# vaibhawvipul/taper

Measured on AMD Instinct MI355X. Metric: MNIST samples/sec fwd+bwd+step, higher is better.
Workload: dtype f32; 1 GPU; mlp_784-128-10_b64; per_gpu_batch=64, global_batch=64, parallelism=single, comm=none, graph_record_steps=11577

## Files before the change

### include/taper_hip.h

```cpp
#ifndef TAPER_HIP_H
#define TAPER_HIP_H

#include <stddef.h>
#include <stdint.h>

#ifdef __cplusplus
extern "C" {
#endif

typedef struct th_ctx th_ctx;
typedef struct th_graph th_graph;
typedef struct th_event th_event;
typedef struct th_comm th_comm;

typedef struct th_adam_fuse {
    float *d_p, *d_m, *d_v;
    const int32_t *d_t;
    const float *d_lr;
    float beta1, beta2, eps, weight_decay;
} th_adam_fuse;

typedef struct th_adam_slice {
    const float *d_g;
    int64_t n;
// ... 44 lines not shown
                  int accumulate_mask);
int th_linear_bwd_adam(th_ctx *ctx, const float *d_x, const float *d_w, const float *d_dy, const float *d_relu_y,
                       float *d_dx, float *d_dw, float *d_db, int batch, int in_features, int out_features,
                       int accumulate_mask, const th_adam_fuse *w_fuse, const th_adam_fuse *b_fuse);
int th_linear_bwd_adam_ex(th_ctx *ctx, const float *d_x, const float *d_w, const float *d_dy, const float *d_relu_y,
                          float *d_dx, float *d_dw, float *d_db, int batch, int in_features, int out_features,
                          int accumulate_mask, const th_adam_fuse *w_fuse, const th_adam_fuse *b_fuse,
                          const th_adam_slice *extra, int n_extra);
int th_linear_bwd_dx_epilogue_rows(int batch, int in_features, int out_features);
int th_linear_bwd_separate_products(int batch, int in_features, int out_features, int with_dx, int with_dw, int dx_epilogue);
int th_linear_bwd_adam_ex2(th_ctx *ctx, const float *d_x, const float *d_w, const float *d_dy, const float *d_relu_y, float *d_dx,
                           float *d_dw, float *d_db, int batch, int in_features, int out_features, int accumulate_mask,
                           const th_adam_fuse *w_fuse, const th_adam_fuse *b_fuse, const th_adam_slice *extra, int n_extra, int mask_dx,
                           float *d_dx_colpart);

int th_linear_xent_head(th_ctx *ctx, const float *d_h, const float *d_w, const float *d_bias, const float *d_targets,
                        int batch, int in_features, int classes, float *d_logits, float *d_loss, float *d_ncorrect,
                        float *d_dh, float *d_dw, float *d_db, float *d_metrics, int64_t metrics_capacity,
                        int64_t *d_state, int64_t advance, int32_t *d_adam_tick, const th_adam_fuse *w_fuse,
                        const th_adam_fuse *b_fuse);
int th_linear_xent_head_masked(th_ctx *ctx, const float *d_h, const float *d_w, const float *d_bias, const float *d_targets,
                               int batch, int in_features, int classes, float *d_logits, float *d_loss, float *d_ncorrect,
                               float *d_dh, float *d_dw, float *d_db, float *d_metrics, int64_t metrics_capacity,
                               int64_t *d_state, int64_t advance, int32_t *d_adam_tick, const th_adam_fuse *w_fuse,
                               const th_adam_fuse *b_fuse, int mask_dh_by_h);

int th_linear_xent_wide(th_ctx *ctx, const float *d_x, const float *d_w, const float *d_bias, const float *d_targets,
                        int batch, int in_features, int classes, float *d_loss, float *d_ncorrect,
                        float *d_dx, float *d_dw, float *d_db, float *d_metrics, int64_t metrics_capacity,
                        int64_t *d_state, int64_t advance, int32_t *d_adam_tick);
int th_linear_xent_wide_ex(th_ctx *ctx, const float *d_x, const float *d_w, const float *d_bias, const float *d_targets, int batch,
                           int in_features, int classes, float *d_loss, float *d_ncorrect, float *d_dx, float *d_dw, float *d_db,
                           float *d_metrics, int64_t metrics_capacity, int64_t *d_state, int64_t advance, int32_t *d_adam_tick,
                           float *d_colsum_masked);
int th_bias_from_colsum_adam(th_ctx *ctx, const float *d_colsum, float *d_gb, int c, int hw, const th_adam_fuse *b_fuse,
                             const th_adam_slice *extra, int n_extra);
typedef struct th_wide_fuse {
    th_adam_fuse w, b, conv_b;
    float *d_conv_gb;
    int conv_c, conv_hw;
} th_wide_fuse;
int th_linear_xent_wide_fused(th_ctx *ctx, const float *d_x, const float *d_w, const float *d_bias, const float *d_targets, int batch,
                              int in_features, int classes, float *d_loss, float *d_ncorrect, float *d_dw, float *d_db,
                              float *d_metrics, int64_t metrics_capacity, int64_t *d_state, int64_t advance, int32_t *d_adam_tick,
                              float *d_colsum_masked, const th_wide_fuse *fuse);

int th_mlp_tail_supported(int batch, int in_features, int hidden, int classes, int need_dx);
int th_mlp_tail(th_ctx *ctx, const float *d_x, const float *d_h, const float *d_w2, const float *d_b2,
                const float *d_targets, int batch, int in_features, int hidden, int classes,
                float *d_loss, float *d_ncorrect, float *d_dw1, float *d_db1, float *d_dw2, float *d_db2,
                const float *d_w1, float *d_dx,
                float *d_metrics, int64_t metrics_capacity, int64_t *d_state, int64_t advance,
                const th_adam_fuse *w1_fuse, const th_adam_fuse *b1_fuse);

typedef struct th_mlp3_layer {
    const float *d_w, *d_b;
    float *d_dw, *d_db;
    const th_adam_fuse *w_fuse, *b_fuse;
    int out_features;
} th_mlp3_layer;
typedef struct th_mlp3_gap {
    const float *d_cnt;
    float *d_gb;
    int hw;
    const th_adam_fuse *b_fuse;
} th_mlp3_gap;
int th_mlp3_supported(int batch, int in_features, int h1, int h2, int classes);
int th_mlp3_xent(th_ctx *ctx, const float *d_x, const float *d_targets, int batch, int in_features, const th_mlp3_layer *layers,
                 float *d_dx, float *d_loss, float *d_ncorrect, float *d_metrics, int64_t metrics_capacity, int64_t *d_state,
                 int64_t advance, int32_t *d_tick, const th_mlp3_gap *gap);

typedef struct th_row_source {
    const float *d_rows;
    const float *d_labels;
    const int32_t *d_indices;
    const int64_t *d_cursor;
    int64_t n_indices;
    int64_t n_rows;
} th_row_source;
int th_mlp2_xent_supported(int batch, int in_features, int hidden, int classes, int64_t n_rows);
int th_mlp2_set_max_ksplit(th_ctx *ctx, int max_ksplit);
int th_mlp2_xent(th_ctx *ctx, const th_row_source *src, int batch, int in_features, int hidden, int classes, const float *d_w1,
                 const float *d_b1, const float *d_w2, const float *d_b2, float *d_dw1, float *d_db1, float *d_dw2, float *d_db2,
                 float *d_loss, float *d_ncorrect, float *d_metrics, int64_t metrics_capacity, int64_t *d_state, int64_t advance,
                 int32_t *d_tick, const th_adam_fuse *w1_fuse, const th_adam_fuse *b1_fuse, const th_adam_fuse *w2_fuse,
                 const th_adam_fuse *b2_fuse);

int th_mlp2_xent_deep_supported(int batch, int in_features, int h1, int h2, int classes, int64_t n_rows);
int th_mlp2_xent_deep(th_ctx *ctx, const th_row_source *src, int batch, int in_features, const th_mlp3_layer *layers, float *d_loss,
                      float *d_ncorrect, float *d_metrics, int64_t metrics_capacity, int64_t *d_state, int64_t advance, int32_t *d_tick);

int th_add(th_ctx *ctx, const float *d_a, const float *d_b, float *d_out, size_t n);
int th_sub(th_ctx *ctx, const float *d_a, const float *d_b, float *d_out, size_t n);
int th_mul(th_ctx *ctx, const float *d_a, const float *d_b, float *d_out, size_t n);
int th_div(th_ctx *ctx, const float *d_a, const float *d_b, float *d_out, size_t n);
int th_axpy(th_ctx *ctx, float alpha, const float *d_x, float *d_y, size_t n);
int th_mul_bwd(th_ctx *ctx, const float *d_gout, const float *d_other, float *d_g, size_t n);
int th_div_bwd(th_ctx *ctx, const float *d_gout, const float *d_a, const float *d_b, float *d_ga, float *d_gb, size_t n);
int th_add_scalar_dev(th_ctx *ctx, const float *d_scalar, float divisor, float *d_g, size_t n);

int th_relu_fwd(th_ctx *ctx, const float *d_x, float *d_y, size_t n);
int th_relu_bwd(th_ctx *ctx, const float *d_x, const float *d_gout, float *d_gin, size_t n, int accumulate);
int th_sigmoid_fwd(th_ctx *ctx, const float *d_x, float *d_y, size_t n);
int th_sigmoid_bwd(th_ctx *ctx, const float *d_y, const float *d_gout, float *d_gin, size_t n);
int th_exp_fwd(th_ctx *ctx, const float *d_x, float *d_y, size_t n);
int th_log_fwd(th_ctx *ctx, const float *d_x, float *d_y, size_t n);
// ... 234 lines not shown
```

### taper_amd/csrc/common.h

```cpp
#pragma once

#include <hip/hip_runtime.h>

#include <cstdarg>
#include <cstdint>
#include <cstdio>
#include <array>
#include <atomic>
#include <map>
#include <string>
#include <unordered_map>
#include <unordered_set>
#include <vector>

#include "../../include/taper_hip.h"
#include "../../include/taper_hip_debug.h"

namespace th {

void set_error(const char *fmt, ...);

#define TH_HIP(expr)                                                                         \
    do {                                                                                     \
        hipError_t e_ = (expr);                                                              \
// ... 35 lines not shown
constexpr int kNumCU = 256;
constexpr int kNumXCD = 8;

static inline int ceil_div(long a, long b) { return (int)((a + b - 1) / b); }

__device__ __forceinline__ void lds_barrier() {
    __builtin_amdgcn_fence(__ATOMIC_RELEASE, "workgroup", "local");
    __builtin_amdgcn_s_barrier();
    __builtin_amdgcn_fence(__ATOMIC_ACQUIRE, "workgroup", "local");
}

enum : int32_t { TH_DEVERR_NONE = 0, TH_DEVERR_TARGET_OOB = 1 };
static __device__ __attribute__((unused)) int32_t *g_err_word;
__device__ __forceinline__ void raise_target_oob(long cls, int classes) {
    int32_t *w = g_err_word;
    if (!w) return;
    w[1] = (int32_t)(cls > 0x7fffffffL ? 0x7fffffffL : cls);
    w[2] = classes;
    __threadfence_system();
    w[0] = TH_DEVERR_TARGET_OOB;
}
typedef int (*err_bind_fn)(int32_t *);
struct ErrBindReg { explicit ErrBindReg(err_bind_fn f); };
#define TH_USES_DEVICE_ERRORS()                                                                                        \
    namespace {                                                                                                        \
    int th_err_bind_here(int32_t *p) { return hipMemcpyToSymbol(HIP_SYMBOL(th::g_err_word), &p, sizeof(p)) == hipSuccess ? 0 : 1; } \
    th::ErrBindReg th_err_reg_here(th_err_bind_here);                                                                  \
    }

static inline int ew_grid(size_t n_items, int block) {
    long g = (long)((n_items + block - 1) / block);
    long cap = (long)kNumCU * 8;
    return (int)(g < 1 ? 1 : (g > cap ? cap : g));
}

}

struct th_ctx {
    int device = 0;
    hipStream_t stream = nullptr;
    std::multimap<size_t, void *> free_blocks;
    std::unordered_map<void *, size_t> block_size;
    std::unordered_set<void *> graph_owned;
    std::unordered_set<void *> graph_owned_freed;
    size_t bytes_reserved = 0, bytes_in_use = 0;
    bool capturing = false;
    std::vector<void *> capture_blocks;
    std::multimap<size_t, void *> capture_free;
    std::map<std::array<int, 8>, void *> conv_plans;
    int32_t *err_word = nullptr;
    int m2_max_ksplit = 8;
    const uint32_t *update_guard = nullptr;
    uint32_t *update_step_word = nullptr;
    unsigned *m2_arrive = nullptr;
};

struct th_graph {
    th_ctx *ctx = nullptr;
    hipGraph_t graph = nullptr;
    hipGraphExec_t exec = nullptr;
    std::vector<void *> blocks;
};

struct th_event {
    hipEvent_t ev = nullptr;
};
```

### taper_amd/csrc/host/taper.h

```cpp
#pragma once

#include <algorithm>
#include <cstdint>
#include <functional>
#include <map>
#include <memory>
#include <random>
#include <stdexcept>
#include <string>
#include <vector>

#include "../../../include/taper_hip.h"

namespace taper {

struct Error : std::runtime_error {
    explicit Error(const std::string &m) : std::runtime_error(m) {}
};
void th_check(int rc, const char *what);
#define TAPER_ASSERT(cond, msg)                       \
    do {                                              \
        if (!(cond)) throw ::taper::Error(msg);       \
    } while (0)

// ... 787 lines not shown
};

struct Metrics {
    std::vector<float> train_loss, train_acc, val_loss, val_acc, epoch_times;
    std::string last_line() const;
    std::string summary() const;
    void print_last() const;
    void plot_summary() const;
};

std::string format_f32_display(float v);

enum class StepForm { Mlp2Rows, ChainMlp3, Mlp3, ChainHead, MlpTail, LinearHead, LinearWide, Layered };
struct StepPlan {
    StepForm form = StepForm::Layered;
    size_t prefix = 0;
    Linear *linear[3] = {};
    std::vector<ConvStage> stages;
    bool fused_adam = false;
    bool pool_bias = false;
    bool conv_chain = false;
    bool exchange = false;
    void key(std::vector<uintptr_t> *out) const;
};

class Trainer {
   public:
    std::shared_ptr<Module> model;
    std::shared_ptr<Adam> optimizer;
    std::shared_ptr<Communicator> comm;
    Shape sample_shape;
    std::string device = "hip:gfx950";
    size_t graph_chunk = 128;
    int fuse_head = 2;
    bool fuse_adam = true;
    Trainer(std::shared_ptr<Module> m, std::shared_ptr<Adam> o) : model(std::move(m)), optimizer(std::move(o)) {}

    void train_step(const Tensor &images, const Tensor &labels, float *loss_out, float *acc_out);
    void check_comm() const;
    void check_batchnorm_comm() const;
    EpochResult train_epoch(DataLoader &loader);
    EpochResult evaluate(DataLoader &loader);
    EpochResult train_epoch_graph(DataLoader &loader, size_t max_steps = 0);
    std::shared_ptr<LRScheduler> scheduler;
    Metrics metrics;
    void fit(DataLoader &train_loader, DataLoader &val_loader, size_t epochs, bool verbose, bool graph = true);
    void save_checkpoint(const std::string &path) const;
    void load_checkpoint(const std::string &path);
    void save_optimizer_state(const std::string &path) const;
    void load_optimizer_state(const std::string &path);
    ~Trainer();

   private:
    void enqueue_steps(const float *d_images, const float *d_labels, const int32_t *d_indices, int64_t n_indices,
                       size_t batch, size_t steps);
    void enqueue_compute(const StepPlan &plan, float *d_xb, float *d_yb, size_t batch, const th_row_source *rows = nullptr);
    StepPlan plan_step(size_t batch, int64_t n_rows) const;
    void drop_graphs();
    std::vector<std::pair<size_t, th_graph *>> graphs_;
    std::vector<std::pair<size_t, th_graph *>> whole_graphs_;
    bool graph_capture_failed_ = false;
    std::vector<size_t> whole_capture_failed_;
    std::vector<uintptr_t> graph_key_;
    std::shared_ptr<Buffer> xb_, yb_, state_, metrics_, step_loss_, step_ncorrect_;
    QATWeightPass qat_pass_;
    bool has_qat() const;
    size_t metrics_cap_ = 0;
};

}
```

### taper_amd/csrc/host/trainer.cpp

```cpp
#include <algorithm>
#include <chrono>
#include <cmath>
#include <cstdio>
#include <cstdlib>
#include <cstring>
#include <fstream>

#include "nn_internal.h"
#include "../../../include/taper_hip_debug.h"

namespace taper {
MNISTDataset MNISTDataset::from_host(const std::vector<float> &images, const std::vector<float> &labels, bool train) {
    TAPER_ASSERT(images.size() == labels.size() * 784, "MNISTDataset: images must be [N,784]");
    MNISTDataset d;
    d.images = Tensor(images, {labels.size(), 784});
    d.labels = Tensor(labels, {labels.size()});
    d.train = train;
    return d;
}

MNISTDataset MNISTDataset::from_u8(const std::vector<uint8_t> &pixels, const std::vector<uint8_t> &labels, bool train) {
    TAPER_ASSERT(pixels.size() == labels.size() * 784, "MNISTDataset: pixels must be [N,784]");
    th_ctx *ctx = Device::ctx();
    MNISTDataset d;
// ... 334 lines not shown
            for (Linear *l : plan.linear)
                if (l) {
                    w.push_back(l->weight);
                    b.push_back(l->bias);
                }
            loss = mlp2_cross_entropy(*rows, batch, w, b, &ncorrect, &sink);
            break;
        }
        case StepForm::ChainMlp3:
        case StepForm::Mlp3: {
            const Tensor w3[3] = {L[0]->weight, L[1]->weight, L[2]->weight}, b3[3] = {L[0]->bias, L[1]->bias, L[2]->bias};
            loss = plan.form == StepForm::ChainMlp3 ? conv_chain_mlp3_cross_entropy(xin, plan.stages, w3, b3, y, &ncorrect, &sink)
                                                    : mlp3_cross_entropy(seq->forward_prefix(xin, plan.prefix), w3, b3, y, &ncorrect, &sink);
            break;
        }
        case StepForm::ChainHead:
            loss = conv_chain_head_cross_entropy(xin, plan.stages, L[0]->weight, L[0]->bias, y, &ncorrect, &sink);
            break;
        case StepForm::MlpTail: {
            Tensor xh = seq->forward_prefix(xin, plan.prefix);
            if (plan.fused_adam) adam->set_carry_deferred(true);
            loss = mlp_tail_cross_entropy(xh, L[0]->weight, L[0]->bias, L[1]->weight, L[1]->bias, y, &ncorrect, &sink);
            break;
        }
        case StepForm::LinearHead:
        case StepForm::LinearWide: {
            adam->flush_deferred();
            Tensor h = seq->forward_prefix(xin, plan.prefix);
            loss = plan.form == StepForm::LinearHead ? linear_cross_entropy(h, L[0]->weight, L[0]->bias, y, &ncorrect, &sink)
                                                     : linear_cross_entropy_wide(h, L[0]->weight, L[0]->bias, y, &ncorrect, &sink);
            break;
        }
        case StepForm::Layered: {
            adam->flush_deferred();
            qat_pass_.run(*model);
            Tensor h = seq ? seq->forward_prefix(xin, plan.prefix) : model->forward(xin);
            for (size_t i = plan.prefix; seq && i < seq->layers.size(); ++i) h = seq->layers[i]->forward(h);
            loss = cross_entropy_loss(h, y, &ncorrect, &sink);
            break;
        }
    }
    loss.backward();
    if (plan.exchange) {
        optimizer->step();
    } else if (!(comm && optimizer->step_reduced(*comm))) {
        reduce_grads(*this);
        optimizer->step();
        optimizer->set_step_guard(nullptr);
    }
    optimizer->zero_grad();
    adam->set_carry_deferred(false);
}

void Trainer::enqueue_steps(const float *d_images, const float *d_labels, const int32_t *d_indices, int64_t n_indices,
                            size_t batch, size_t steps) {
    int64_t *state = reinterpret_cast<int64_t *>(state_->d);
    struct Guard {
        Guard(const uint32_t *w, uint32_t *step) { TH(th_ctx_set_update_guard(Device::ctx(), w, step)); }
        ~Guard() { th_ctx_set_update_guard(Device::ctx(), nullptr, nullptr); }
    } guard(comm && comm->is_p2p() ? comm->error_word() : nullptr, comm && comm->is_p2p() ? comm->step_word() : nullptr);
    const StepPlan plan = plan_step(batch, d_indices ? n_indices : (int64_t)batch);
    if (plan.form == StepForm::Mlp2Rows) {
        const th_row_source rows{d_images, d_labels, d_indices, d_indices ? state + 1 : nullptr, d_indices ? n_indices : 0,
                                 d_indices ? n_indices : (int64_t)batch};
        for (size_t s = 0; s < steps; ++s) enqueue_compute(plan, nullptr, nullptr, batch, &rows);
    } else if (d_indices == nullptr) {
        enqueue_compute(plan, const_cast<float *>(d_images), const_cast<float *>(d_labels), batch);
    } else {
        TH(th_gather_batch(Device::ctx(), d_images, d_labels, d_indices, n_indices, state + 1, (int)(batch * steps), 784, xb_->d,
                           yb_->d));
        for (size_t s = 0; s < steps; ++s) enqueue_compute(plan, xb_->d + s * batch * 784, yb_->d + s * batch, batch);
    }
    optimizer->flush_deferred();
}

void Trainer::check_batchnorm_comm() const {
    if (!comm) return;
    std::vector<BatchNorm2d *> bns;
    batchnorm_modules(*model, &bns);
    TAPER_ASSERT(bns.empty(), "BatchNorm2d: data-parallel training of a model with batch normalisation is not supported (statistics are per rank)");
}

bool Trainer::has_qat() const {
    std::vector<const QATModule *> mods;
    qat_modules(*model, &mods, false);
    for (size_t i = 0; i < mods.size(); ++i)
        for (size_t j = i + 1; j < mods.size(); ++j)
            TAPER_ASSERT(mods[i] != mods[j], "QAT: the model holds the same QAT layer twice; the Trainer does not train a shared QAT layer");
    return !mods.empty();
}

void Trainer::drop_graphs() {
    for (auto &g : graphs_) th_graph_destroy(g.second);
    graphs_.clear();
    for (auto &g : whole_graphs_) th_graph_destroy(g.second);
    whole_graphs_.clear();
    whole_capture_failed_.clear();
}

EpochResult Trainer::train_epoch_graph(DataLoader &loader, size_t max_steps) {
    th_ctx *ctx = Device::ctx();
    static const bool trace = std::getenv("TAPER_TRACE_EPOCH") != nullptr;
    const auto t_enter = std::chrono::steady_clock::now();
    auto us_since = [&](std::chrono::steady_clock::time_point t0) { return std::chrono::duration<double, std::micro>(std::chrono::steady_clock::now() - t0).count(); };
    loader.reset();
    const MNISTDataset &ds = loader.dataset();
    const size_t n = ds.len(), bs = loader.batch_size();
    size_t nb = loader.num_batches();
    if (max_steps && max_steps < nb) nb = max_steps;
    const size_t n_full = std::min(nb, n / bs);
    const size_t rem_rows = nb > n_full ? n - n_full * bs : 0;
    const StepPlan plan = plan_step(bs, (int64_t)n), rem_plan = rem_rows ? plan_step(rem_rows, (int64_t)n) : StepPlan{};
    const bool full_in_place = plan.form == StepForm::Mlp2Rows;
    const size_t chunk = full_in_place ? std::max<size_t>(graph_chunk, 1) : std::max<size_t>(std::min<size_t>(graph_chunk, ((size_t)1 << 26) / (bs * 784)), 1);
    const float *d_img = ds.images.dptr(), *d_lab = ds.labels.dptr();
    const int32_t *d_idx = (!loader.shuffled() && bs >= n && nb == 1) ? nullptr : loader.d_indices();
    const size_t stage_rows = std::max(full_in_place ? (size_t)0 : chunk * bs, (rem_rows && rem_plan.form != StepForm::Mlp2Rows) ? rem_rows : (size_t)0);
    if (d_idx && stage_rows && (!xb_ || xb_->n < stage_rows * 784)) {
        drop_graphs();
        xb_ = Buffer::alloc(stage_rows * 784);
        yb_ = Buffer::alloc(stage_rows);
    }
    if (!state_) state_ = Buffer::alloc(4);
    if (metrics_cap_ < loader.num_batches() + 1) {
        drop_graphs();
        metrics_cap_ = loader.num_batches() + 1;
        metrics_ = Buffer::alloc_host(2 * metrics_cap_);
    }
    std::vector<uintptr_t> key{(uintptr_t)d_img, (uintptr_t)d_lab, (uintptr_t)d_idx, (uintptr_t)n, (uintptr_t)bs, (uintptr_t)comm.get(),
                               (uintptr_t)model.get(), (uintptr_t)optimizer.get(), (uintptr_t)optimizer->flat().p_arena->d,
                               (uintptr_t)optimizer->flat().g_arena->d, (uintptr_t)(xb_ ? xb_->d : nullptr), (uintptr_t)metrics_->d};
    plan.key(&key);
    for (size_t d : sample_shape) key.push_back((uintptr_t)d);
    for (float h : {optimizer->beta1(), optimizer->beta2(), optimizer->eps(), optimizer->weight_decay()}) {
        uint32_t bits;
        std::memcpy(&bits, &h, sizeof bits);
        key.push_back(bits);
    }
    key.push_back((uintptr_t)full_backward());
    {
        uintptr_t h = 1469598103934665603ull;
        for (const Tensor &p : optimizer->flat().params) h = (h ^ (uintptr_t)(p.get_requires_grad() ? 2 : 1)) * 1099511628211ull;
        key.push_back(h);
    }
    {
        std::vector<const QATModule *> mods, active;
        qat_modules(*model, &mods, false);
        qat_modules(*model, &active, true);
        if (!mods.empty()) {
            qat_pass_.sync(active);
            key.push_back((uintptr_t)qat::enabled() | (uintptr_t)qat::is_training() << 1);
            key.push_back((uintptr_t)qat_pass_.generation());
        }
        for (const QATModule *q : mods)
            key.push_back((uintptr_t)q->active() | (uintptr_t)q->config.activations << 1 | (uintptr_t)q->config.qtype << 2);
    }
    {
        std::vector<BatchNorm2d *> bns;
        batchnorm_modules(*model, &bns);
        for (const BatchNorm2d *b : bns) key.push_back((uintptr_t)0xb0 | (uintptr_t)b->is_training());
    }
    if (!graphs_.empty() && graph_key_ != key) drop_graphs();

    size_t done = 0;
    th_graph *whole = nullptr;
    if (nb == n_full && !graph_capture_failed_ && !(std::getenv("TAPER_NO_GRAPH") && std::getenv("TAPER_NO_GRAPH")[0] == '1'))
        for (auto &g : whole_graphs_)
            if (g.first == n_full) whole = g.second;
    const double us_prep = us_since(t_enter);
    if (!whole) TH(th_fill_f32(ctx, state_->d, 0.f, 4));
    const double us_fill = us_since(t_enter);
    if (whole) {
        TH(th_graph_launch(ctx, whole));
        done = n_full;
    }
    auto have = [&](size_t steps) {
        for (auto &g : graphs_)
            if (g.first == steps) return true;
        return false;
    };
    if (!graph_capture_failed_ && std::getenv("TAPER_NO_GRAPH") && std::getenv("TAPER_NO_GRAPH")[0] == '1') graph_capture_failed_ = true;
    if (comm && !graph_capture_failed_ && std::getenv("TAPER_DP_EAGER") && std::getenv("TAPER_DP_EAGER")[0] == '1')
        graph_capture_failed_ = true;
    std::vector<size_t> want;
    for (size_t steps = chunk;; steps /= 2) {
        if (steps < 1) steps = 1;
        if (!((steps > 1 && n_full < steps + 1) || have(steps)) && std::find(want.begin(), want.end(), steps) == want.end())
            want.push_back(steps);
        if (steps == 1) break;
    }
    if (!whole && !want.empty() && n_full > 0 && !graph_capture_failed_) {
        enqueue_steps(d_img, d_lab, d_idx, (int64_t)n, bs, 1);
        done = 1;
        for (size_t steps : want) {
            TH(th_graph_begin(ctx));
            th_graph *g = nullptr;
            try {
                enqueue_steps(d_img, d_lab, d_idx, (int64_t)n, bs, steps);
                TH(th_graph_end(ctx, &g));
            } catch (const std::exception &e) {
                if (!g) th_graph_end(ctx, &g);
                if (g) th_graph_destroy(g);
                if (!comm) throw;
                fprintf(stderr, "taper: step capture with the communicator failed (%s); running data-parallel steps eagerly\n", e.what());
                graph_capture_failed_ = true;
                break;
            }
            graphs_.emplace_back(steps, g);
        }
        std::sort(graphs_.begin(), graphs_.end(), [](const auto &x, const auto &y) { return x.first > y.first; });
        graph_key_ = key;
    }
    if (!whole) {
        const size_t tail = n_full - done > 0 ? (n_full - done) % chunk : 0;
        size_t exact = 0;
        for (auto &g : graphs_) exact += (g.first & (g.first - 1)) != 0 ? 1 : 0;
        if (tail > 2 && (tail & (tail - 1)) != 0 && !have(tail) && have(1) && exact < 4 && !graph_capture_failed_ &&
            graph_key_ == key) {
            TH(th_graph_begin(ctx));
            th_graph *g = nullptr;
            try {
                enqueue_steps(d_img, d_lab, d_idx, (int64_t)n, bs, tail);
                TH(th_graph_end(ctx, &g));
                graphs_.emplace_back(tail, g);
                std::sort(graphs_.begin(), graphs_.end(), [](const auto &x, const auto &y) { return x.first > y.first; });
            } catch (const std::exception &e) {
                fprintf(stderr, "taper: capturing a %zu-step remainder graph failed (%s); the ladder graphs serve it\n", tail, e.what());
                if (!g) th_graph_end(ctx, &g);
                if (g) th_graph_destroy(g);
                if (auto *adam = dynamic_cast<Adam *>(optimizer.get())) {
                    adam->set_carry_deferred(false);
                    adam->drop_step_bookkeeping();
                }
                optimizer->zero_grad();
                Tape::reset();
                if (!comm) throw;
            }
        }
    }
    if (!whole && done == 0 && nb == n_full && n_full >= 2 && have(n_full) && whole_graphs_.size() < 4 && !graph_capture_failed_ && graph_key_ == key &&
        std::find(whole_capture_failed_.begin(), whole_capture_failed_.end(), n_full) == whole_capture_failed_.end()) {
        TH(th_graph_begin(ctx));
        th_graph *g = nullptr;
        try {
            TH(th_fill_f32(ctx, state_->d, 0.f, 4));
            enqueue_steps(d_img, d_lab, d_idx, (int64_t)n, bs, n_full);
            TH(th_graph_end(ctx, &g));
            whole_graphs_.emplace_back(n_full, g);
            TH(th_graph_launch(ctx, g));
            done = n_full;
        } catch (const std::exception &e) {
            fprintf(stderr, "taper: capturing a whole-call graph of %zu steps failed (%s); reset + replay stay two launches\n", n_full, e.what());
            whole_capture_failed_.push_back(n_full);
            if (!g) th_graph_end(ctx, &g);
            if (g) th_graph_destroy(g);
            if (auto *adam = dynamic_cast<Adam *>(optimizer.get())) {
                adam->set_carry_deferred(false);
                adam->drop_step_bookkeeping();
            }
            optimizer->zero_grad();
            Tape::reset();
            if (!comm) throw;
        }
    }
    while (done < n_full) {
        bool launched = false;
        for (auto &g : graphs_) {
            if (done + g.first <= n_full) {
                TH(th_graph_launch(ctx, g.second));
                done += g.first;
                launched = true;
                break;
            }
        }
        if (!launched) {
            enqueue_steps(d_img, d_lab, d_idx, (int64_t)n, bs, 1);
            ++done;
        }
    }
    if (nb > n_full) {
        const size_t rem = n - n_full * bs;
        enqueue_steps(d_img, d_lab, d_idx, (int64_t)n, rem, 1);
    }
    loader.advance(std::min(n, nb * bs));

    const double us_enqueued = us_since(t_enter);
    Device::sync();
    check_comm();
    if (trace) fprintf(stderr, "taper trace: train_epoch_graph %zu steps (%s%s%s): state reset enqueued at %.1f - %.1f us, all enqueued after %.1f us, stream idle after %.1f us\n", nb,
                       step_form_names[(int)plan.form], rem_rows ? ", last batch " : "", rem_rows ? step_form_names[(int)rem_plan.form] : "", us_prep, us_fill, us_enqueued, us_since(t_enter));
    const float *mt = metrics_->d;
    EpochResult r;
    r.num_batches = nb;
    float total_loss = 0.f;
    for (size_t s = 0; s < nb; ++s) {
        const size_t b = (s < n_full) ? bs : n - n_full * bs;
        const float acc = mt[2 * s + 1] / (float)b;
        r.total_correct += (size_t)(acc * (float)b);
        r.total_samples += b;
// ... 13 lines not shown
```

### taper_amd/csrc/mlp_tail.hip

```cpp
#include "tail_dev.h"
#include "dp_dev.h"

TH_USES_DEVICE_ERRORS()

namespace th {

struct TailArgs {
    const float *x, *h, *w2, *b2, *targets;
    int batch, in_f, hid, c;
    float *loss, *ncorrect, *dw1, *db1, *dw2, *db2;
    float *metrics;
    int64_t capacity;
    int64_t *state;
    int64_t advance;
    AdamDev w1_adam, b1_adam;
    int n_dw, n_head, tiles_m, groups;
    const float *w1;
    float *dx;
    int xgroups;
    DpDev dp;
    int32_t *dp_tick;
};

#ifdef TH_PROFILE
__device__ long long g_tail_prof[2][16];
#define TAIL_STAMP(i)                                                                         \
    do {                                                                                      \
        __builtin_amdgcn_sched_barrier(0);                                                    \
        if (threadIdx.x == 0 && (blockIdx.x == 0 || blockIdx.x == a.n_head))                  \
            g_tail_prof[blockIdx.x == 0 ? 0 : 1][i] = wall_clock64();                         \
        __builtin_amdgcn_sched_barrier(0);                                                    \
    } while (0)
__global__ void tail_prof_mark_kernel(int i) { g_tail_prof[0][i] = g_tail_prof[1][i] = wall_clock64(); }
#else
#define TAIL_STAMP(i) do { } while (0)
#endif

template <int KS, int TN>
__global__ __launch_bounds__(256) void mlp_tail_kernel(TailArgs a) {
    __shared__ float red[4][TN][64][4];
    __shared__ float tr[4][16][17];
    __shared__ float sc[4][36];
    const int t = threadIdx.x, lane = t & 63, wave = t >> 6, r16 = lane & 15, g4 = lane >> 4;
    const int bid = blockIdx.x;
    TAIL_STAMP(0);
    const bool head_role = bid < a.n_head;
    int tile_m, grp = 0;
    if (!head_role) {
        const int b2 = bid - a.n_head;
        const int tt = (b2 & 7) * (a.n_dw >> 3) + (b2 >> 3);
        if (tt >= a.tiles_m * a.groups) return;
        tile_m = tt % a.tiles_m;
        grp = tt / a.tiles_m;
    } else {
        tile_m = bid;
        if (tile_m >= a.tiles_m) return;
    }
    const int hid = a.hid, C = a.c, in_f = a.in_f, B = a.batch;
    const int hcol = tile_m * 16 + r16;
    const bool hcol_ok = hcol < hid;
    const int col0 = grp * 16 * TN;
    const bool lead = head_role && tile_m == 0;

    const bool any_w = a.w1_adam.p != nullptr, any_b = a.db1 && a.b1_adam.p != nullptr;
    const int32_t w_t = any_w ? sload(a.w1_adam.t) : 1, b_t = any_b ? sload(a.b1_adam.t) : 1;
    const float w_lr = any_w ? sload(a.w1_adam.lr) : 0.f, b_lr = any_b ? sload(a.b1_adam.lr) : 0.f;
    const int Cm1 = C - 1, hid4 = hid - 4, hcol_c = min(hcol, hid - 1);
// ... 277 lines not shown
    float lg[4], dl[4], nll_row;
    int bi;
#pragma unroll
    for (int i = 0; i < 4; ++i) lg[i] = (g4 * 4 + i < C) ? ((ax[i] + ay[i]) + (az[i] + aw[i])) + b2v[i] : -INFINITY;
    tail_row_softmax(lg, g4, C, tf, 1.0f / (float)B, dl, nll_row, bi);

    floatx4 accx[TX];
#pragma unroll
    for (int tx = 0; tx < TX; ++tx) accx[tx] = floatx4{0.f, 0.f, 0.f, 0.f};
#pragma unroll
    for (int th0 = 0; th0 < KS; th0 += TH_BLK) {
        float w2t[TH_BLK][4], w1v[TH_BLK][TX][4];
#pragma unroll
        for (int t = 0; t < TH_BLK; ++t)
#pragma unroll
            for (int s = 0; s < 4; ++s) {
                w2t[t][s] = ldg_b(a.w2, cls_off[s] + (th0 + t) * 64);
#pragma unroll
                for (int tx = 0; tx < TX; ++tx)
                    w1v[t][tx][s] = tx_ok[tx] ? ldg_b(a.w1, w1_off + ((th0 + t) * 16 + s) * in_f * 4u + tx * 64) : 0.f;
            }
#pragma unroll
        for (int t = 0; t < TH_BLK; ++t) {
            floatx4 dht = {0.f, 0.f, 0.f, 0.f};
#pragma unroll
            for (int s = 0; s < 4; ++s) dht = __builtin_amdgcn_mfma_f32_16x16x4f32(w2t[t][s], dl[s], dht, 0, 0, 0);
            const float4 hq = hv[th0 + t];
            const float m[4] = {hq.x > 0.f ? dht[0] : 0.f, hq.y > 0.f ? dht[1] : 0.f, hq.z > 0.f ? dht[2] : 0.f, hq.w > 0.f ? dht[3] : 0.f};
#pragma unroll
            for (int s = 0; s < 4; ++s)
#pragma unroll
                for (int tx = 0; tx < TX; ++tx) accx[tx] = __builtin_amdgcn_mfma_f32_16x16x4f32(m[s], w1v[t][tx][s], accx[tx], 0, 0, 0);
        }
    }
    const unsigned x_off = ((unsigned)(r0 + g4 * 4) * in_f + col0 + r16) * 4u;
#pragma unroll
    for (int tx = 0; tx < TX; ++tx) {
        if (!tx_ok[tx]) continue;
#pragma unroll
        for (int i = 0; i < 4; ++i) *reinterpret_cast<float *>(reinterpret_cast<char *>(a.dx) + x_off + i * in_f * 4u + tx * 64) = accx[tx][i];
    }
}

template <int KS, int TN, bool HAS_DX, int NW, int DPNR = 0>
__global__ __launch_bounds__(64 * NW) void mlp_tail_exact_kernel(TailArgs a) {
    constexpr unsigned HID = 16 * KS;
    __shared__ float red[NW][TN][64][4];
    __shared__ float tr[NW][16][17];
    __shared__ float rowv[NW][2][16];
    __shared__ float sc[NW][36];
    asm volatile("" ::"s"(a.x), "s"(a.h), "s"(a.w2), "s"(a.b2), "s"(a.targets), "s"(a.batch), "s"(a.in_f), "s"(a.c), "s"(a.dw1),
                 "s"(a.db1), "s"(a.w1_adam.p), "s"(a.w1_adam.m), "s"(a.w1_adam.v), "s"(a.w1_adam.t), "s"(a.w1_adam.lr),
                 "s"(a.b1_adam.p), "s"(a.b1_adam.t), "s"(a.b1_adam.lr), "s"(a.n_dw), "s"(a.n_head), "s"(a.groups), "s"(a.metrics),
                 "s"(a.state));
    const int t = threadIdx.x, lane = t & 63, wave = t >> 6, r16 = lane & 15, g4 = lane >> 4;
    const int bid = blockIdx.x;
    TAIL_STAMP(0);
    DpTicket dp_tk{0u, 0u};
    if constexpr (DPNR > 0) dp_tk = dp_begin(a.dp);
    if (HAS_DX && bid >= a.n_head + a.n_dw) {
        tail_dx_role<KS, NW>(a, bid - a.n_head - a.n_dw);
        return;
    }
    const bool head_role = bid < a.n_head;
    int tile_m, grp = 0, tt = 0;
    if (!head_role) {
        const int b2 = bid - a.n_head;
        tt = (b2 & 7) * (a.n_dw >> 3) + (b2 >> 3);
        if (tt >= KS * a.groups) return;
        tile_m = tt % KS;
        grp = tt / KS;
    } else {
        tile_m = bid;
        if (tile_m >= KS) return;
    }
    const int C = a.c, B = a.batch;
    const unsigned in_f = (unsigned)a.in_f;
    const unsigned hcol = tile_m * 16 + r16;
    const unsigned col0 = grp * 16 * TN;
    const bool lead = head_role && tile_m == 0;
    const bool any_w = a.w1_adam.p != nullptr, any_b = a.db1 && a.b1_adam.p != nullptr;
    const int32_t w_t = any_w ? sload(a.w1_adam.t) : 1, b_t = any_b ? sload(a.b1_adam.t) : 1;
    const float w_lr = any_w ? sload(a.w1_adam.lr) : 0.f, b_lr = any_b ? sload(a.b1_adam.lr) : 0.f;

    float4 wv[KS];
    const unsigned w_off = ((unsigned)min(r16, C - 1) * HID + g4 * 4) * 4u;
#pragma unroll
    for (int ks = 0; ks < KS; ++ks) wv[ks] = ldg4_b(a.w2, w_off + ks * 64);
    float w2b[4], b2v[4];
#pragma unroll
    for (int s = 0; s < 4; ++s) {
        const unsigned cls = (unsigned)min(g4 * 4 + s, C - 1);
        w2b[s] = ldg_b(a.w2, (cls * HID + hcol) * 4u);
        b2v[s] = a.b2 ? ldg_b(a.b2, cls * 4u) : 0.f;
    }
    bool tn_ok[TN];
#pragma unroll
    for (int tn = 0; tn < TN; ++tn) tn_ok[tn] = col0 + tn * 16 < in_f;
    const unsigned e_off = ((tile_m * 16 + g4 * 4 + wave) * in_f + col0 + r16) * 4u;
    const bool fuse_w = !head_role && any_w;
    const bool finisher = NW == 4 || wave < 4;
    float e_p[TN], e_m[TN], e_v[TN], w_step = 0.f, b_step = 0.f;
#pragma unroll
    for (int tn = 0; tn < TN; ++tn) {
        e_p[tn] = e_m[tn] = e_v[tn] = 0.f;
        if (fuse_w && tn_ok[tn] && finisher) {
            e_p[tn] = ldg_b(a.w1_adam.p, e_off + tn * 64);
            e_m[tn] = ldg_b(a.w1_adam.m, e_off + tn * 64);
            e_v[tn] = ldg_b(a.w1_adam.v, e_off + tn * 64);
        }
    }
    const bool fuse_b1 = head_role && any_b;
    const unsigned b1_off = (tile_m * 16 + (t & 15)) * 4u;
    float bp_ = 0.f, bm_ = 0.f, bv_ = 0.f;
    if (fuse_b1) {
        bp_ = ldg_b(a.b1_adam.p, b1_off);
        bm_ = ldg_b(a.b1_adam.m, b1_off);
        bv_ = ldg_b(a.b1_adam.v, b1_off);
    }
    const int64_t state0 = (lead && a.metrics) ? sload(a.state) : 0, state1 = (lead && a.metrics) ? sload(a.state + 1) : 0;

    floatx4 accdw[TN];
#pragma unroll
    for (int tn = 0; tn < TN; ++tn) accdw[tn] = floatx4{0.f, 0.f, 0.f, 0.f};
    floatx4 acc_dw2 = {0.f, 0.f, 0.f, 0.f};
    float db1_acc = 0.f, db2_acc = 0.f, nll_acc = 0.f, hit_acc = 0.f;
    const float inv_b = 1.0f / (float)B;

    float4 hv[KS];
    float tf = 0.f, hm[4], xv[TN][4];
    auto load_chunk = [&](int c0) {
        const int r0 = c0 + wave * 16;
        if (r0 >= B) return;
        const unsigned h_off = ((unsigned)(r0 + r16) * HID + g4 * 4) * 4u;
#pragma unroll
        for (int ks = 0; ks < KS; ++ks) hv[ks] = ldg4_b(a.h, h_off + ks * 64);
        tf = ldg_b(a.targets, (unsigned)(r0 + r16) * 4u);
        const unsigned hm_off = ((unsigned)(r0 + g4 * 4) * HID + hcol) * 4u;
        const unsigned x_off = ((unsigned)(r0 + g4 * 4) * in_f + col0 + r16) * 4u;
#pragma unroll
        for (int s = 0; s < 4; ++s) {
            hm[s] = ldg_b(a.h, hm_off + s * HID * 4);
#pragma unroll
            for (int tn = 0; tn < TN; ++tn)
                xv[tn][s] = (!head_role && tn_ok[tn]) ? ldg_b(a.x, x_off + s * in_f * 4u + tn * 64) : 0.f;
        }
    };
    load_chunk(0);
    TAIL_STAMP(1);
    if (fuse_w) w_step = adam_step_size(w_lr, a.w1_adam.beta1, a.w1_adam.beta2, w_t);
    if (fuse_b1) b_step = adam_step_size(b_lr, a.b1_adam.beta1, a.b1_adam.beta2, b_t);
    TAIL_STAMP(2);

    for (int c0 = 0;;) {
        const int r0 = c0 + wave * 16;
        const bool rows_here = r0 < B;
        if (rows_here) {
            TAIL_STAMP(3);
            floatx4 ax = {0.f, 0.f, 0.f, 0.f}, ay = ax, az = ax, aw = ax;
#pragma unroll
            for (int ks = 0; ks < KS; ++ks) {
                ax = __builtin_amdgcn_mfma_f32_16x16x4f32(wv[ks].x, hv[ks].x, ax, 0, 0, 0);
                ay = __builtin_amdgcn_mfma_f32_16x16x4f32(wv[ks].y, hv[ks].y, ay, 0, 0, 0);
                az = __builtin_amdgcn_mfma_f32_16x16x4f32(wv[ks].z, hv[ks].z, az, 0, 0, 0);
                aw = __builtin_amdgcn_mfma_f32_16x16x4f32(wv[ks].w, hv[ks].w, aw, 0, 0, 0);
            }
            float lg[4], dl[4], nll_row;
            int bi;
#pragma unroll
            for (int i = 0; i < 4; ++i) lg[i] = (g4 * 4 + i < C) ? ((ax[i] + ay[i]) + (az[i] + aw[i])) + b2v[i] : -INFINITY;
            tail_row_softmax(lg, g4, C, tf, inv_b, dl, nll_row, bi);
            TAIL_STAMP(4);

// ... 148 lines not shown
        const int ix = tile_m * 16 + t;
        a.db1[ix] = out;
        if (fuse_b1) {
            const AdamDev &ad = a.b1_adam;
            const float gv = out + ad.wd * bp_;
            const float mn = ad.beta1 * bm_ + (1.0f - ad.beta1) * gv;
            const float vn = ad.beta2 * bv_ + (1.0f - ad.beta2) * gv * gv;
            ad.m[ix] = mn;
            ad.v[ix] = vn;
            ad.p[ix] = bp_ - b_step * mn / (sqrtf(vn) + ad.eps);
        }
    }
    if (lead) {
        if (DPNR == 0 && a.db2 && t < C) {
            float sum = sc[0][16 + t];
#pragma unroll
            for (int w = 1; w < NW; ++w) sum += sc[w][16 + t];
            a.db2[t] = sum;
        }
        if (t == 0) {
            float n = sc[0][32], hsum = sc[0][33];
#pragma unroll
            for (int w = 1; w < NW; ++w) {
                n += sc[w][32];
                hsum += sc[w][33];
            }
            const float l = n / (float)B;
            a.loss[0] = l;
            if (a.ncorrect) a.ncorrect[0] = hsum;
            if (a.metrics) {
                const int64_t log_slot = state0 < a.capacity ? state0 : state0 % a.capacity;
                a.metrics[2 * log_slot] = l;
                a.metrics[2 * log_slot + 1] = hsum;
                a.state[0] = state0 + 1;
                a.state[1] = state1 + a.advance;
            }
        }
    }
    TAIL_STAMP(7);
}

}

using namespace th;

static bool tail_whole_tiles(int batch, int in_features, int hidden) {
    return (hidden == 32 || hidden == 64 || hidden == 128 || hidden == 256) && batch % 16 == 0 && in_features % 16 == 0;
}

extern "C" int th_mlp_tail_supported(int batch, int in_features, int hidden, int classes, int need_dx) {
    const bool ok = batch > 0 && batch <= 512 && in_features > 0 && hidden > 0 && hidden <= 256 && (hidden % 4) == 0 && classes > 0 &&
                    classes <= 16;
    return ok && (!need_dx || tail_whole_tiles(batch, in_features, hidden));
}

static bool tail_dp_shapes(int batch, int in_features, int hidden, int classes) {
    return th_mlp_tail_supported(batch, in_features, hidden, classes, 0) && tail_whole_tiles(batch, in_features, hidden) &&
           (hidden == 64 || hidden == 128);
}
static int tail_dp_grid(int in_features, int hidden) {
    const int tiles_m = hidden / 16, groups = ceil_div(in_features, 32);
    return ((tiles_m * groups + 7) & ~7) + ((tiles_m + 7) & ~7);
}
template <int KS, int NW>
static const void *tail_dp_instance(int n_ranks) {
    if (n_ranks <= 2) return (const void *)mlp_tail_exact_kernel<KS, 2, false, NW, 2>;
    if (n_ranks <= 4) return (const void *)mlp_tail_exact_kernel<KS, 2, false, NW, 4>;
    return (const void *)mlp_tail_exact_kernel<KS, 2, false, NW, 8>;
}
static const void *tail_dp_kernel(int batch, int hidden, int n_ranks) {
    const bool nw8 = batch > 64;
    if (hidden == 64) return nw8 ? tail_dp_instance<4, 8>(n_ranks) : tail_dp_instance<4, 4>(n_ranks);
    return nw8 ? tail_dp_instance<8, 8>(n_ranks) : tail_dp_instance<8, 4>(n_ranks);
}

extern "C" int th_mlp_tail_dp_supported(const th_comm *comm, th_ctx *ctx, int batch, int in_features, int hidden, int classes) {
    const DpDev *dp = comm_dp_dev(comm);
    if (!dp || !ctx || dp->n_ranks < 2 || !tail_dp_shapes(batch, in_features, hidden, classes)) return 0;
    const int grid = tail_dp_grid(in_features, hidden);
    if (grid > DP_MAX_SLOTS) return 0;
    if (comm_dp_sharing(comm) > 1) {
        int per_cu = 0;
        if (hipOccupancyMaxActiveBlocksPerMultiprocessor(&per_cu, tail_dp_kernel(batch, hidden, dp->n_ranks), batch > 64 ? 512 : 256, 0) != hipSuccess) {
            (void)hipGetLastError();
            return 0;
        }
        if (!comm_dp_shared_fits(comm, grid, per_cu)) return 0;
    }
    return 1;
}

static int mlp_tail_launch(th_comm *comm, th_ctx *ctx, const float *d_x, const float *d_h, const float *d_w2, const float *d_b2,
                           const float *d_targets, int batch, int in_features, int hidden, int classes, float *d_loss,
                           float *d_ncorrect, float *d_dw1, float *d_db1, float *d_dw2, float *d_db2, const float *d_w1, float *d_dx,
                           float *d_metrics, int64_t metrics_capacity, int64_t *d_state, int64_t advance,
                           const th_adam_fuse *w1_fuse, const th_adam_fuse *b1_fuse, int32_t *d_tick) {
    TH_REQUIRE(ctx && d_x && d_h && d_w2 && d_targets && d_loss && d_dw1, "th_mlp_tail: null argument");
    TH_REQUIRE(th_mlp_tail_supported(batch, in_features, hidden, classes, 0),
               "th_mlp_tail: needs batch <= 512, hidden <= 256 and a multiple of 4, classes <= 16 (got %d, %d, %d)", batch, hidden, classes);
    TH_REQUIRE(!d_dx || (d_w1 && tail_whole_tiles(batch, in_features, hidden)),
               "th_mlp_tail: d_dx needs d_w1 and whole tiles (hidden 32 / 64 / 128 / 256, batch and in_features multiples of 16)");
    TH_REQUIRE(!d_dx || !(w1_fuse && w1_fuse->d_p), "th_mlp_tail: with d_dx the launch reads W1, its update must be deferred (th_adam_slice)");
    TH_REQUIRE((((uintptr_t)d_h | (uintptr_t)d_w2) & 15) == 0, "th_mlp_tail: d_h and d_w2 must be 16-byte aligned");
    TH_REQUIRE(!d_metrics || (d_state && metrics_capacity > 0), "th_mlp_tail: metrics need d_state and a capacity");
    TH_REQUIRE(!(b1_fuse && b1_fuse->d_p) || d_db1, "th_mlp_tail: fused b1 update needs d_db1");
    constexpr int TN = 2;
    TailArgs a{};
    a.x = d_x; a.h = d_h; a.w2 = d_w2; a.b2 = d_b2; a.targets = d_targets;
    a.batch = batch; a.in_f = in_features; a.hid = hidden; a.c = classes;
    a.loss = d_loss; a.ncorrect = d_ncorrect; a.dw1 = d_dw1; a.db1 = d_db1; a.dw2 = d_dw2; a.db2 = d_db2;
    a.metrics = d_metrics; a.capacity = metrics_capacity; a.state = d_state; a.advance = advance;
    a.w1_adam = make_adam_dev(w1_fuse);
    a.b1_adam = make_adam_dev(b1_fuse);
    a.tiles_m = ceil_div(hidden, 16);
    a.groups = ceil_div(in_features, 16 * TN);
    a.n_dw = (a.tiles_m * a.groups + 7) & ~7;
    a.n_head = (a.tiles_m + 7) & ~7;
    a.w1 = d_w1;
    a.dx = d_dx;
    a.xgroups = ceil_div(in_features, 32);
    const int nw = batch <= 64 ? 4 : 8;
    const int grid = a.n_dw + a.n_head + (d_dx ? a.xgroups * ceil_div(batch, 16 * nw) : 0);
    const bool exact = tail_whole_tiles(batch, in_features, hidden);
    if (comm) {
        const DpDev *dp = comm_dp_dev(comm);
        TH_REQUIRE(dp && th_mlp_tail_dp_supported(comm, ctx, batch, in_features, hidden, classes),
                   "th_mlp_tail_dp: this communicator / shape cannot take the in-launch exchange (th_mlp_tail_dp_supported)");
        TH_REQUIRE(!d_dx && exact && grid == tail_dp_grid(in_features, hidden), "th_mlp_tail_dp: internal: launch shape");
        a.dp = *dp;
        a.dp_tick = d_tick;
        const void *fn = tail_dp_kernel(batch, hidden, dp->n_ranks);
        void *args[] = {&a};
        TH_HIP(hipLaunchKernel(fn, dim3(grid), dim3(64 * nw), args, 0, ctx->stream));
        comm_dp_count_launch(comm);
        return 0;
    }
#define TH_TAIL_LAUNCH(KS)                                                                                            \
    do {                                                                                                              \
        if (exact && d_dx && nw == 8) hipLaunchKernelGGL((mlp_tail_exact_kernel<KS, TN, true, 8>), dim3(grid), dim3(512), 0, ctx->stream, a);     \
        else if (exact && d_dx) hipLaunchKernelGGL((mlp_tail_exact_kernel<KS, TN, true, 4>), dim3(grid), dim3(256), 0, ctx->stream, a);     \
        else if (exact && nw == 8) hipLaunchKernelGGL((mlp_tail_exact_kernel<KS, TN, false, 8>), dim3(grid), dim3(512), 0, ctx->stream, a);     \
        else if (exact) hipLaunchKernelGGL((mlp_tail_exact_kernel<KS, TN, false, 4>), dim3(grid), dim3(256), 0, ctx->stream, a);     \
        else hipLaunchKernelGGL((mlp_tail_kernel<KS, TN>), dim3(grid), dim3(256), 0, ctx->stream, a);                 \
    } while (0)
    if (exact && hidden == 32) TH_TAIL_LAUNCH(2);
    else if (hidden <= 64) TH_TAIL_LAUNCH(4);
    else if (hidden <= 128) TH_TAIL_LAUNCH(8);
    else TH_TAIL_LAUNCH(16);
#undef TH_TAIL_LAUNCH
    TH_LAUNCH_CHECK();
    return 0;
}

extern "C" int th_mlp_tail(th_ctx *ctx, const float *d_x, const float *d_h, const float *d_w2, const float *d_b2,
                           const float *d_targets, int batch, int in_features, int hidden, int classes, float *d_loss,
                           float *d_ncorrect, float *d_dw1, float *d_db1, float *d_dw2, float *d_db2, const float *d_w1, float *d_dx,
                           float *d_metrics, int64_t metrics_capacity, int64_t *d_state, int64_t advance,
                           const th_adam_fuse *w1_fuse, const th_adam_fuse *b1_fuse) {
    return mlp_tail_launch(nullptr, ctx, d_x, d_h, d_w2, d_b2, d_targets, batch, in_features, hidden, classes, d_loss, d_ncorrect, d_dw1, d_db1,
                           d_dw2, d_db2, d_w1, d_dx, d_metrics, metrics_capacity, d_state, advance, w1_fuse, b1_fuse, nullptr);
}

extern "C" int th_mlp_tail_dp(th_comm *comm, th_ctx *ctx, const float *d_x, const float *d_h, const float *d_w2, const float *d_b2,
                              const float *d_targets, int batch, int in_features, int hidden, int classes, float *d_loss,
// ... 20 lines not shown
```

### taper_amd/csrc/runtime.hip

```cpp
#include "common.h"

#include <cstring>

namespace th {

static thread_local std::string g_last_error;

void set_error(const char *fmt, ...) {
    char buf[1024];
    va_list ap;
    va_start(ap, fmt);
    vsnprintf(buf, sizeof(buf), fmt, ap);
    va_end(ap);
    g_last_error = buf;
}

static std::vector<err_bind_fn> &err_binders() {
    static std::vector<err_bind_fn> v;
    return v;
}
ErrBindReg::ErrBindReg(err_bind_fn f) { err_binders().push_back(f); }
static std::map<int, int32_t *> g_err_blocks;

static int err_block_for(int device, int32_t **out) {
// ... 39 lines not shown
    float4 v4 = make_float4(v, v, v, v);
    float4 *p4 = reinterpret_cast<float4 *>(p);
    for (size_t j = i; j < n4; j += stride) p4[j] = v4;
    for (size_t j = n4 * 4 + i; j < n; j += stride) p[j] = v;
}

}

using namespace th;

extern "C" {

const char *th_last_error(void) { return g_last_error.c_str(); }

int th_device_count(int *out) {
    TH_REQUIRE(out, "th_device_count: null out");
    TH_HIP(hipGetDeviceCount(out));
    return 0;
}

int th_ctx_create(int device_id, th_ctx **out) {
    TH_REQUIRE(out, "th_ctx_create: null out");
    int n = 0;
    TH_HIP(hipGetDeviceCount(&n));
    TH_REQUIRE(device_id >= 0 && device_id < n, "th_ctx_create: device %d not present (%d visible)", device_id, n);
    TH_HIP(hipSetDevice(device_id));
    th_ctx *c = new th_ctx();
    c->device = device_id;
    TH_HIP(hipStreamCreateWithFlags(&c->stream, hipStreamNonBlocking));
    if (err_block_for(device_id, &c->err_word)) return 1;
    TH_HIP(hipMalloc((void **)&c->m2_arrive, 512 * sizeof(unsigned)));
    TH_HIP(hipMemsetAsync(c->m2_arrive, 0, 512 * sizeof(unsigned), c->stream));
    TH_HIP(hipStreamSynchronize(c->stream));
    *out = c;
    return 0;
}

int th_ctx_destroy(th_ctx *ctx) {
    if (!ctx) return 0;
    (void)hipSetDevice(ctx->device);
    (void)hipStreamSynchronize(ctx->stream);
    for (auto &kv : ctx->block_size) (void)hipFree(kv.first);
    for (auto &kv : ctx->conv_plans) (void)hipFree(kv.second);
    if (ctx->m2_arrive) (void)hipFree(ctx->m2_arrive);
    (void)hipStreamDestroy(ctx->stream);
    delete ctx;
    return 0;
}

int th_ctx_set_update_guard(th_ctx *ctx, const uint32_t *d_skip_if_nonzero, uint32_t *d_step_word) {
    TH_REQUIRE(ctx, "th_ctx_set_update_guard: null ctx");
    ctx->update_guard = d_skip_if_nonzero;
    ctx->update_step_word = d_step_word;
    return 0;
}

int th_ctx_sync(th_ctx *ctx) {
    TH_REQUIRE(ctx, "th_ctx_sync: null ctx");
    TH_HIP(hipStreamSynchronize(ctx->stream));
    return err_block_check(ctx);
}

void *th_ctx_stream(th_ctx *ctx) { return ctx ? (void *)ctx->stream : nullptr; }
int th_ctx_device(th_ctx *ctx) { return ctx ? ctx->device : -1; }

int th_malloc(th_ctx *ctx, size_t bytes, void **d_out) {
    TH_REQUIRE(ctx && d_out, "th_malloc: null argument");
    size_t sz = round_size(bytes);
    void *p = nullptr;
    if (ctx->capturing) {
        auto it = ctx->capture_free.find(sz);
        if (it != ctx->capture_free.end()) {
            p = it->second;
            ctx->capture_free.erase(it);
        }
    }
    if (!p) {
        auto it = ctx->free_blocks.find(sz);
        if (it != ctx->free_blocks.end()) {
            p = it->second;
            ctx->free_blocks.erase(it);
        } else {
            TH_HIP(hipSetDevice(ctx->device));
            TH_HIP(hipMalloc(&p, sz));
            ctx->block_size[p] = sz;
            ctx->bytes_reserved += sz;
        }
        if (ctx->capturing) ctx->capture_blocks.push_back(p);
    }
    ctx->bytes_in_use += sz;
    *d_out = p;
    return 0;
}

int th_free(th_ctx *ctx, void *d_ptr) {
    if (!d_ptr) return 0;
    TH_REQUIRE(ctx, "th_free: null ctx");
    auto it = ctx->block_size.find(d_ptr);
    TH_REQUIRE(it != ctx->block_size.end(), "th_free: %p was not allocated by this ctx", d_ptr);
    size_t sz = it->second;
    ctx->bytes_in_use -= sz;
    if (ctx->graph_owned.count(d_ptr)) {
        ctx->graph_owned_freed.insert(d_ptr);
        return 0;
    }
    if (ctx->capturing) {
// ... 160 lines not shown
```

Baseline: 5.223 million samples/s.

## Skip batch gather and state reset when unshuffled MLP tail reads rows in place

When the loader is not shuffled and the step form is the MLP tail, the whole-epoch graph now points each step directly at the dataset rows instead of gathering them into a staging buffer first. The first step of the call can also treat the metrics state as zero instead of loading it, which lets the graph drop its state-clearing fill kernel. This removes a large gather copy and a fill launch per epoch graph. In exchange it adds a per-context flag, more graph-cache key bits and a correctness dependency on the kernel that runs first.

```diff
diff --git a/include/taper_hip.h b/include/taper_hip.h
--- a/include/taper_hip.h
+++ b/include/taper_hip.h
@@ -120,6 +120,8 @@
                 const float *d_w1, float *d_dx,
                 float *d_metrics, int64_t metrics_capacity, int64_t *d_state, int64_t advance,
                 const th_adam_fuse *w1_fuse, const th_adam_fuse *b1_fuse);
+int th_mlp_tail_whole_tiles(int batch, int in_features, int hidden);
+int th_ctx_set_state_origin(th_ctx *ctx, int on);
 
 typedef struct th_mlp3_layer {
     const float *d_w, *d_b;
diff --git a/taper_amd/csrc/common.h b/taper_amd/csrc/common.h
--- a/taper_amd/csrc/common.h
+++ b/taper_amd/csrc/common.h
@@ -111,6 +111,7 @@
     int m2_max_ksplit = 8;
     const uint32_t *update_guard = nullptr;
     uint32_t *update_step_word = nullptr;
+    bool state_origin = false;
     unsigned *m2_arrive = nullptr;
 };
 
diff --git a/taper_amd/csrc/host/taper.h b/taper_amd/csrc/host/taper.h
--- a/taper_amd/csrc/host/taper.h
+++ b/taper_amd/csrc/host/taper.h
@@ -863,8 +863,11 @@
     ~Trainer();
 
    private:
+    struct CallStart { bool shuffled; };
     void enqueue_steps(const float *d_images, const float *d_labels, const int32_t *d_indices, int64_t n_indices,
-                       size_t batch, size_t steps);
+                       size_t batch, size_t steps, const CallStart *call_start = nullptr);
+    bool takes_state_origin(const StepPlan &plan, size_t batch) const;
+    bool reads_rows_in_place(const StepPlan &plan, bool shuffled) const;
     void enqueue_compute(const StepPlan &plan, float *d_xb, float *d_yb, size_t batch, const th_row_source *rows = nullptr);
     StepPlan plan_step(size_t batch, int64_t n_rows) const;
     void drop_graphs();
diff --git a/taper_amd/csrc/host/trainer.cpp b/taper_amd/csrc/host/trainer.cpp
--- a/taper_amd/csrc/host/trainer.cpp
+++ b/taper_amd/csrc/host/trainer.cpp
@@ -410,8 +410,16 @@
     adam->set_carry_deferred(false);
 }
 
+bool Trainer::takes_state_origin(const StepPlan &plan, size_t batch) const {
+    if (plan.form != StepForm::MlpTail || comm) return false;
+    const Tensor &w1 = plan.linear[0]->weight;
+    return th_mlp_tail_whole_tiles((int)batch, (int)w1.shape()[1], (int)w1.shape()[0]) != 0;
+}
+
+bool Trainer::reads_rows_in_place(const StepPlan &plan, bool shuffled) const { return plan.form == StepForm::MlpTail && !comm && !shuffled; }
+
 void Trainer::enqueue_steps(const float *d_images, const float *d_labels, const int32_t *d_indices, int64_t n_indices,
-                            size_t batch, size_t steps) {
+                            size_t batch, size_t steps, const CallStart *call_start) {
     int64_t *state = reinterpret_cast<int64_t *>(state_->d);
     struct Guard {
         Guard(const uint32_t *w, uint32_t *step) { TH(th_ctx_set_update_guard(Device::ctx(), w, step)); }
@@ -425,9 +433,23 @@
     } else if (d_indices == nullptr) {
         enqueue_compute(plan, const_cast<float *>(d_images), const_cast<float *>(d_labels), batch);
     } else {
-        TH(th_gather_batch(Device::ctx(), d_images, d_labels, d_indices, n_indices, state + 1, (int)(batch * steps), 784, xb_->d,
-                           yb_->d));
-        for (size_t s = 0; s < steps; ++s) enqueue_compute(plan, xb_->d + s * batch * 784, yb_->d + s * batch, batch);
+        const bool origin = call_start && takes_state_origin(plan, batch);
+        const bool in_place = call_start && reads_rows_in_place(plan, call_start->shuffled);
+        TAPER_ASSERT(!in_place || (int64_t)(batch * steps) <= n_indices, "enqueue_steps: the call's rows run past the dataset");
+        float *xs = in_place ? const_cast<float *>(d_images) : xb_->d, *ys = in_place ? const_cast<float *>(d_labels) : yb_->d;
+        if (!in_place)
+            TH(th_gather_batch(Device::ctx(), d_images, d_labels, d_indices, n_indices, origin ? nullptr : state + 1, (int)(batch * steps), 784,
+                               xs, ys));
+        struct Origin {
+            explicit Origin(bool on) : on_(on) { if (on_) TH(th_ctx_set_state_origin(Device::ctx(), 1)); }
+            void clear() { if (on_) th_ctx_set_state_origin(Device::ctx(), 0); on_ = false; }
+            ~Origin() { clear(); }
+            bool on_;
+        } latch(origin);
+        for (size_t s = 0; s < steps; ++s) {
+            enqueue_compute(plan, xs + s * batch * 784, ys + s * batch, batch);
+            latch.clear();
+        }
     }
     optimizer->flush_deferred();
 }
@@ -496,6 +518,7 @@
         key.push_back(bits);
     }
     key.push_back((uintptr_t)full_backward());
+    key.push_back((uintptr_t)takes_state_origin(plan, bs) | (uintptr_t)reads_rows_in_place(plan, loader.shuffled()) << 1 | (uintptr_t)loader.shuffled() << 2);
     {
         uintptr_t h = 1469598103934665603ull;
         for (const Tensor &p : optimizer->flat().params) h = (h ^ (uintptr_t)(p.get_requires_grad() ? 2 : 1)) * 1099511628211ull;
@@ -601,8 +624,9 @@
         TH(th_graph_begin(ctx));
         th_graph *g = nullptr;
         try {
-            TH(th_fill_f32(ctx, state_->d, 0.f, 4));
-            enqueue_steps(d_img, d_lab, d_idx, (int64_t)n, bs, n_full);
+            const CallStart start{loader.shuffled()};
+            if (!takes_state_origin(plan, bs)) TH(th_fill_f32(ctx, state_->d, 0.f, 4));
+            enqueue_steps(d_img, d_lab, d_idx, (int64_t)n, bs, n_full, &start);
             TH(th_graph_end(ctx, &g));
             whole_graphs_.emplace_back(n_full, g);
             TH(th_graph_launch(ctx, g));
diff --git a/taper_amd/csrc/mlp_tail.hip b/taper_amd/csrc/mlp_tail.hip
--- a/taper_amd/csrc/mlp_tail.hip
+++ b/taper_amd/csrc/mlp_tail.hip
@@ -13,6 +13,7 @@
     int64_t capacity;
     int64_t *state;
     int64_t advance;
+    int state_origin;
     AdamDev w1_adam, b1_adam;
     int n_dw, n_head, tiles_m, groups;
     const float *w1;
@@ -396,7 +397,7 @@
     asm volatile("" ::"s"(a.x), "s"(a.h), "s"(a.w2), "s"(a.b2), "s"(a.targets), "s"(a.batch), "s"(a.in_f), "s"(a.c), "s"(a.dw1),
                  "s"(a.db1), "s"(a.w1_adam.p), "s"(a.w1_adam.m), "s"(a.w1_adam.v), "s"(a.w1_adam.t), "s"(a.w1_adam.lr),
                  "s"(a.b1_adam.p), "s"(a.b1_adam.t), "s"(a.b1_adam.lr), "s"(a.n_dw), "s"(a.n_head), "s"(a.groups), "s"(a.metrics),
-                 "s"(a.state));
+                 "s"(a.state), "s"(a.state_origin));
     const int t = threadIdx.x, lane = t & 63, wave = t >> 6, r16 = lane & 15, g4 = lane >> 4;
     const int bid = blockIdx.x;
     TAIL_STAMP(0);
@@ -462,7 +463,8 @@
         bm_ = ldg_b(a.b1_adam.m, b1_off);
         bv_ = ldg_b(a.b1_adam.v, b1_off);
     }
-    const int64_t state0 = (lead && a.metrics) ? sload(a.state) : 0, state1 = (lead && a.metrics) ? sload(a.state + 1) : 0;
+    const bool load_state = lead && a.metrics && !a.state_origin;
+    const int64_t state0 = load_state ? sload(a.state) : 0, state1 = load_state ? sload(a.state + 1) : 0;
 
     floatx4 accdw[TN];
 #pragma unroll
@@ -717,6 +719,10 @@
     const bool ok = batch > 0 && batch <= 512 && in_features > 0 && hidden > 0 && hidden <= 256 && (hidden % 4) == 0 && classes > 0 &&
                     classes <= 16;
     return ok && (!need_dx || tail_whole_tiles(batch, in_features, hidden));
+}
+
+extern "C" int th_mlp_tail_whole_tiles(int batch, int in_features, int hidden) {
+    return th_mlp_tail_supported(batch, in_features, hidden, 1, 0) && tail_whole_tiles(batch, in_features, hidden);
 }
 
 static bool tail_dp_shapes(int batch, int in_features, int hidden, int classes) {
@@ -769,12 +775,15 @@
     TH_REQUIRE((((uintptr_t)d_h | (uintptr_t)d_w2) & 15) == 0, "th_mlp_tail: d_h and d_w2 must be 16-byte aligned");
     TH_REQUIRE(!d_metrics || (d_state && metrics_capacity > 0), "th_mlp_tail: metrics need d_state and a capacity");
     TH_REQUIRE(!(b1_fuse && b1_fuse->d_p) || d_db1, "th_mlp_tail: fused b1 update needs d_db1");
+    TH_REQUIRE(!ctx->state_origin || !d_metrics || (!comm && tail_whole_tiles(batch, in_features, hidden)),
+               "th_mlp_tail: only the whole-tile kernel takes the state origin (th_ctx_set_state_origin, th_mlp_tail_whole_tiles)");
     constexpr int TN = 2;
     TailArgs a{};
     a.x = d_x; a.h = d_h; a.w2 = d_w2; a.b2 = d_b2; a.targets = d_targets;
     a.batch = batch; a.in_f = in_features; a.hid = hidden; a.c = classes;
     a.loss = d_loss; a.ncorrect = d_ncorrect; a.dw1 = d_dw1; a.db1 = d_db1; a.dw2 = d_dw2; a.db2 = d_db2;
     a.metrics = d_metrics; a.capacity = metrics_capacity; a.state = d_state; a.advance = advance;
+    a.state_origin = ctx->state_origin ? 1 : 0;
     a.w1_adam = make_adam_dev(w1_fuse);
     a.b1_adam = make_adam_dev(b1_fuse);
     a.tiles_m = ceil_div(hidden, 16);
diff --git a/taper_amd/csrc/runtime.hip b/taper_amd/csrc/runtime.hip
--- a/taper_amd/csrc/runtime.hip
+++ b/taper_amd/csrc/runtime.hip
@@ -115,6 +115,12 @@
     TH_REQUIRE(ctx, "th_ctx_set_update_guard: null ctx");
     ctx->update_guard = d_skip_if_nonzero;
     ctx->update_step_word = d_step_word;
+    return 0;
+}
+
+int th_ctx_set_state_origin(th_ctx *ctx, int on) {
+    TH_REQUIRE(ctx, "th_ctx_set_state_origin: null ctx");
+    ctx->state_origin = on != 0;
     return 0;
 }
 
```

Measured after the change: 5.149 million samples/s. 1.4% lower.
